# OpenGVLab/MM-Interleaved

Measured on NVIDIA H100. Metric: interleaved_steps_per_sec, higher is better.
Workload: dtype bf16

## Files before the change

### include/mmfs_b200.h

```cpp
#ifndef MMFS_B200_H_
#define MMFS_B200_H_

#include <stdint.h>

#ifdef __cplusplus
extern "C" {
#endif

#define MMFS_B200_ABI_VERSION 3

#define MMFS_OK            0
#define MMFS_EINVAL       (-1)
#define MMFS_EUNSUPPORTED (-2)
#define MMFS_ECUDA        (-3)

#define MMFS_F32  0
#define MMFS_F16  1
#define MMFS_BF16 2
#define MMFS_F64  3

#define MMFS_MSDA_STRICT 1u

#define MMFS_SAMPLER_EXACT_WEIGHTS 4u
#define MMFS_SAMPLER_GENERIC       8u
// ... 124 lines not shown
                       const float *params, const int64_t *seed, const float *uniforms, int B, int V, int max_new,
                       int mode, void *stream);

int mmfs_beam_select(const float *logits, long ld, const int64_t *step, const double *params, float *beam_scores,
                     int64_t *history, int64_t *next_ids, int64_t *parent, uint8_t *done, double *hyp_scores,
                     int64_t *hyp_ids, int64_t *hyp_meta, const int64_t *eos_ids, int n_eos, long pad_id, int min_length,
                     uint64_t *scratch, int B, int num_beams, int V, int max_new, void *stream);

int mmfs_beam_sample(const float *logits, long ld, const int64_t *step, const double *params, const int64_t *seed,
                     const float *uniforms, float *beam_scores, int64_t *history, int64_t *next_ids, int64_t *parent,
                     uint8_t *done, double *hyp_scores, int64_t *hyp_ids, int64_t *hyp_meta, int32_t *error,
                     const int64_t *eos_ids, int n_eos, long pad_id, int min_length, int top_k, uint64_t *scratch, int B,
                     int num_beams, int V, int max_new, void *stream);

int mmfs_kv_beam_reorder(void *cache, int n_caches, long cache_stride, int rows, long row_stride, long pos_stride,
                         long row_bytes, int num_beams, const int64_t *parent, const int64_t *cur, const int64_t *step,
                         const uint8_t *done, int max_positions, void *stream);

int mmfs_image_reentry(const float *images, float *out, int N, int C, int H, int W, int R, void *stream);

int mmfs_linear_fp8(const void *x, const uint8_t *w8, const float *scale, const void *bias, const void *residual,
                    void *out, int M, int N, int K, int dtype, void *stream);

#ifdef __cplusplus
}
#endif
#endif
```

### mm-interleaved_b200/_lib.py

```python
from __future__ import annotations

import ctypes
import os

_HERE = os.path.dirname(os.path.abspath(__file__))
LIB_PATH = os.environ.get("MMFS_B200_LIB", os.path.join(_HERE, "libmmfs_b200.so"))

OK, EINVAL, EUNSUPPORTED, ECUDA = 0, -1, -2, -3
F32, F16, BF16, F64 = 0, 1, 2, 3
MSDA_STRICT = 1
SAMPLER_EXACT_WEIGHTS = 4
SAMPLER_GENERIC = 8
SELECT_GREEDY, SELECT_SAMPLE = 0, 1

_lib = None

_I, _U, _P = ctypes.c_int, ctypes.c_uint, ctypes.c_void_p
_L, _F = ctypes.c_long, ctypes.c_float

SIGNATURES = {
    "mmfs_abi_version": (_I, []),
    "mmfs_last_error": (ctypes.c_char_p, []),
    "mmfs_msda_forward": (_I, [_P, _P, _P, _P, _P, _P, _I, _I, _I, _I, _I, _I, _I, _I, _U, _P]),
    "mmfs_msda_backward": (_I, [_P] * 9 + [_I] * 8 + [_P]),
# ... 13 lines not shown
    "mmfs_groupnorm_nhwc": (_I, [_P] * 5 + [_I] * 4 + [_F, _I, _I, _P]),
    "mmfs_groupnorm_nhwc_backward": (_I, [_P] * 6 + [_I] * 4 + [_F, _I, _I, _P]),
    "mmfs_conv2d_nhwc": (_I, [_P] * 6 + [_I] * 10 + [_P]),
    "mmfs_conv2d_up2x_nhwc": (_I, [_P] * 4 + [_I] * 6 + [_P]),
    "mmfs_conv2d_down2x_nhwc": (_I, [_P] * 4 + [_I] * 6 + [_P]),
    "mmfs_attn_decode_scratch_floats": (_L, [_I] * 4),
    "mmfs_attn_decode": (_I, [_P] * 6 + [_I] * 4 + [_L] * 6 + [_F, _I, _I, _I, _P]),
    "mmfs_attn_forward": (_I, [_P] * 5 + [_I] * 5 + [_L] * 8 + [_F, _I, _I, _I, _P, _P]),
    "mmfs_attn_forward_lse": (_I, [_P] * 6 + [_I] * 5 + [_L] * 8 + [_F, _I, _I, _I, _P, _P]),
    "mmfs_attn_backward": (_I, [_P] * 11 + [_I] * 4 + [_L] * 16 + [_F, _I, _P]),
    "mmfs_attn_backward_general": (_I, [_P] * 11 + [_I] * 5 + [_L] * 16 + [_F, _I, _I, _P]),
    "mmfs_rmsnorm_backward": (_I, [_P] * 6 + [_L, _I, _F, _I, _P]),
    "mmfs_layernorm_backward": (_I, [_P] * 7 + [_L, _I, _F, _I, _P]),
    "mmfs_swiglu_backward": (_I, [_P] * 3 + [_L, _I, _I, _P]),
    "mmfs_geglu_backward": (_I, [_P] * 3 + [_L, _I, _I, _P]),
    "mmfs_quick_gelu_backward": (_I, [_P] * 3 + [_L, _I, _P]),
    "mmfs_resize_bilinear_backward": (_I, [_P] * 2 + [_I] * 6 + [_L] * 3 + [_F, _F, _I, _P]),
    "mmfs_decode_select": (_I, [_P, _L] + [_P] * 5 + [_I, _L, _I] + [_P] * 3 + [_I] * 4 + [_P]),
    "mmfs_beam_select": (_I, [_P, _L] + [_P] * 11 + [_I, _L, _I, _P] + [_I] * 4 + [_P]),
    "mmfs_beam_sample": (_I, [_P, _L] + [_P] * 14 + [_I, _L, _I, _I, _P] + [_I] * 4 + [_P]),
    "mmfs_kv_beam_reorder": (_I, [_P, _I, _L, _I, _L, _L, _L, _I] + [_P] * 4 + [_I, _P]),
    "mmfs_image_reentry": (_I, [_P, _P] + [_I] * 5 + [_P]),
    "mmfs_linear_fp8": (_I, [_P] * 6 + [_I] * 4 + [_P]),
}
BEAM_MAX_BEAMS, BEAM_MAX_EOS = 8, 4
LINEAR_FP8_MAX_M = 64
RMSNORM_BWD_PARTS = 256


def lib() -> ctypes.CDLL:
    global _lib
    if _lib is None:
        if not os.path.exists(LIB_PATH):
            raise RuntimeError(
                f"libmmfs_b200.so not found at {LIB_PATH}: build it with "
                "`python mm-interleaved_b200/build.py` (there is no CPU / PyTorch fallback)")
        handle = ctypes.CDLL(LIB_PATH)
        for name, (res, args) in SIGNATURES.items():
            fn = getattr(handle, name)
            fn.restype = res
            fn.argtypes = args
        if handle.mmfs_abi_version() != 3:
            raise RuntimeError(f"libmmfs_b200.so ABI {handle.mmfs_abi_version()} != 3")
        _lib = handle
    return _lib

# ... 7 lines not shown
```

### mm-interleaved_b200/csrc/common.cuh

```cuda
#pragma once
#include <cuda_bf16.h>
#include <cuda_fp16.h>
#include <cuda_runtime.h>
#include <stdint.h>
#include <stdio.h>

#include <type_traits>

#include "../../include/mmfs_b200.h"

namespace mmfs {

void set_error(const char *fmt, ...);
int cuda_fail(cudaError_t e, const char *what);

#define MMFS_CHECK_ARG(cond, ...)            \
    do {                                     \
        if (!(cond)) {                       \
            ::mmfs::set_error(__VA_ARGS__);  \
            return MMFS_EINVAL;              \
        }                                    \
    } while (0)

#define MMFS_CUDA(call)                                             \
// ... 43 lines not shown
    MMFS_CUDA(cudaFuncSetAttribute(Kernel, cudaFuncAttributeMaxDynamicSharedMemorySize, (int)bytes));
    if (tracked) set[dev] = bytes;
    return MMFS_OK;
}

inline int capped_grid(long blocks, int per_sm) {
    const long cap = (long)num_sms() * per_sm;
    return (int)(blocks < cap ? blocks : cap);
}

template <typename T> struct OpMath { using type = float; };
template <> struct OpMath<double> { using type = double; };

__device__ __forceinline__ float to_op(float x) { return x; }
__device__ __forceinline__ double to_op(double x) { return x; }
__device__ __forceinline__ float to_op(__half x) { return __half2float(x); }
__device__ __forceinline__ float to_op(__nv_bfloat16 x) { return __bfloat162float(x); }

template <typename T> __device__ __forceinline__ T from_op(typename OpMath<T>::type x);
template <> __device__ __forceinline__ float from_op<float>(float x) { return x; }
template <> __device__ __forceinline__ double from_op<double>(double x) { return x; }
template <> __device__ __forceinline__ __half from_op<__half>(float x) { return __float2half_rn(x); }
template <> __device__ __forceinline__ __nv_bfloat16 from_op<__nv_bfloat16>(float x) { return __float2bfloat16_rn(x); }

template <typename T> struct Vec16;
template <> struct Vec16<float> {
    static constexpr int N = 4;
    __device__ __forceinline__ static void unpack(const uint4 &v, float (&f)[4]) {
        f[0] = __uint_as_float(v.x); f[1] = __uint_as_float(v.y);
        f[2] = __uint_as_float(v.z); f[3] = __uint_as_float(v.w);
    }
    __device__ __forceinline__ static uint4 pack(const float (&f)[4]) {
        return make_uint4(__float_as_uint(f[0]), __float_as_uint(f[1]), __float_as_uint(f[2]), __float_as_uint(f[3]));
    }
};
template <> struct Vec16<__nv_bfloat16> {
    static constexpr int N = 8;
    __device__ __forceinline__ static void unpack(const uint4 &v, float (&f)[8]) {
        f[0] = __uint_as_float(v.x << 16); f[1] = __uint_as_float(v.x & 0xffff0000u);
        f[2] = __uint_as_float(v.y << 16); f[3] = __uint_as_float(v.y & 0xffff0000u);
        f[4] = __uint_as_float(v.z << 16); f[5] = __uint_as_float(v.z & 0xffff0000u);
        f[6] = __uint_as_float(v.w << 16); f[7] = __uint_as_float(v.w & 0xffff0000u);
    }
    __device__ __forceinline__ static uint4 pack(const float (&f)[8]) {
        uint4 r;
        __nv_bfloat162 a = __floats2bfloat162_rn(f[0], f[1]); r.x = *reinterpret_cast<uint32_t *>(&a);
// ... 78 lines not shown
```

### mm-interleaved_b200/csrc/conv_igemm_sm100.cu

```cuda
#include "tc_common.cuh"

namespace mmfs {

constexpr int kConvStages = 4;
constexpr int kConvThreads = 288;
constexpr int kConvConsumers = 256;

struct ConvParams {
    void *out;
    const void *bias, *add_bc, *residual;
    int B, Ho, Wo, Cin, Cout, KH, KW, stride, pad;
    int TW, TH, TB;
    int tiles_w, tiles_h;
};

template <typename T> __device__ __forceinline__ uint32_t cpack2(float a, float b);
template <> __device__ __forceinline__ uint32_t cpack2<__nv_bfloat16>(float a, float b) {
    __nv_bfloat162 t = __floats2bfloat162_rn(a, b);
    return *reinterpret_cast<uint32_t *>(&t);
}
template <> __device__ __forceinline__ uint32_t cpack2<__half>(float a, float b) {
    __half2 t = __floats2half2_rn(a, b);
    return *reinterpret_cast<uint32_t *>(&t);
}
template <typename T> __device__ __forceinline__ float2 cunpack2(const T *p);
template <> __device__ __forceinline__ float2 cunpack2<__nv_bfloat16>(const __nv_bfloat16 *p) {
    return __bfloat1622float2(*reinterpret_cast<const __nv_bfloat162 *>(p));
}
template <> __device__ __forceinline__ float2 cunpack2<__half>(const __half *p) {
    return __half22float2(*reinterpret_cast<const __half2 *>(p));
}

template <typename T, int BN, bool UP>
__global__ void __launch_bounds__(kConvThreads, 1)
conv_igemm_kernel(const __grid_constant__ CUtensorMap map_x, const __grid_constant__ CUtensorMap map_w, const ConvParams p) {
    static_assert(BN == 160 || BN == 128, "Cout tile");
    constexpr uint32_t A_BYTES = 128 * 128, B_BYTES = BN * 128, STAGE_BYTES = A_BYTES + B_BYTES;
    extern __shared__ __align__(1024) uint8_t smem_raw[];
    if ((s_addr(smem_raw) & 1023u) != 0u) { asm volatile("trap;"); }
    uint64_t *bars = reinterpret_cast<uint64_t *>(smem_raw + kConvStages * STAGE_BYTES);
    uint64_t *full = bars, *empty = bars + kConvStages;

    const int warp = threadIdx.x >> 5, lane = threadIdx.x & 31;
    int t = blockIdx.x;
    const int wt = t % p.tiles_w; t /= p.tiles_w;
    const int ht = t % p.tiles_h; t /= p.tiles_h;
    const int b0 = t * p.TB, h0 = ht * p.TH, w0 = wt * p.TW;
// ... 181 lines not shown
```

### mm-interleaved_b200/csrc/llama_ops_sm100.cu

```cuda
#include "common.cuh"

namespace mmfs {

template <typename T> __device__ __forceinline__ float rnd(float x) { return to_op(from_op<T>(x)); }
template <> __device__ __forceinline__ float rnd<float>(float x) { return x; }

__device__ __forceinline__ float block_sum(float v, float *s_red) {
#pragma unroll
    for (int o = 16; o > 0; o >>= 1) v += __shfl_xor_sync(0xffffffffu, v, o);
    const int lane = threadIdx.x & 31, warp = threadIdx.x >> 5, nw = (blockDim.x + 31) >> 5;
    if (lane == 0) s_red[warp] = v;
    __syncthreads();
    float t = (lane < nw) ? s_red[lane] : 0.f;
#pragma unroll
    for (int o = 16; o > 0; o >>= 1) t += __shfl_xor_sync(0xffffffffu, t, o);
    __syncthreads();
    return t;
}

template <typename T>
__global__ void __launch_bounds__(256) rmsnorm_kernel(const T *__restrict__ x, const T *__restrict__ w,
                                                       T *__restrict__ y, int cols, float eps) {
    constexpr int VEC = 16 / (int)sizeof(T);
    __shared__ float s_red[32];
    const size_t row = blockIdx.x;
    const T *xr = x + row * cols;
    T *yr = y + row * cols;
    const int nvec = cols / VEC;
// ... 222 lines not shown
            const T *src = (is_k ? kt + (size_t)(hh - H) * hd : qt + (size_t)hh * hd) + c * VEC;
            T *dst = (is_k ? kc + (size_t)(hh - H) * hd : qt + (size_t)hh * hd) + c * VEC;
            float cs[VEC], sn[VEC], x1[VEC], x2[VEC], o1[VEC], o2[VEC];
#pragma unroll
            for (int i = 0; i < VEC; i += 4) {
                const float4 a = *reinterpret_cast<const float4 *>(cp + c * VEC + i);
                const float4 bb = *reinterpret_cast<const float4 *>(sp + c * VEC + i);
                cs[i] = rnd<T>(a.x); cs[i + 1] = rnd<T>(a.y); cs[i + 2] = rnd<T>(a.z); cs[i + 3] = rnd<T>(a.w);
                sn[i] = rnd<T>(bb.x); sn[i + 1] = rnd<T>(bb.y); sn[i + 2] = rnd<T>(bb.z); sn[i + 3] = rnd<T>(bb.w);
            }
            Vec16<T>::unpack(*reinterpret_cast<const uint4 *>(src), x1);
            Vec16<T>::unpack(*reinterpret_cast<const uint4 *>(src + half), x2);
#pragma unroll
            for (int i = 0; i < VEC; ++i) {
                o1[i] = rnd<T>(x1[i] * cs[i]) + rnd<T>(-x2[i] * sn[i]);
                o2[i] = rnd<T>(x2[i] * cs[i]) + rnd<T>(x1[i] * sn[i]);
            }
            *reinterpret_cast<uint4 *>(dst) = Vec16<T>::pack(o1);
            *reinterpret_cast<uint4 *>(dst + half) = Vec16<T>::pack(o2);
        }
    }
}

template <typename T> __device__ __forceinline__ float silu_op(float g) { return __fdividef(g, 1.f + __expf(-g)); }
template <> __device__ __forceinline__ float silu_op<float>(float g) { return g / (1.f + expf(-g)); }

template <typename T, int ACT> __device__ __forceinline__ float glu_act(float g) {
    if (ACT == 0) return silu_op<T>(g);
    return 0.5f * g * (1.f + erff(g * 0.70710678118654752f));
}

template <typename T, int ACT = 0, bool GATE_SECOND = false>
__global__ void __launch_bounds__(256) swiglu_kernel(const T *__restrict__ gu, T *__restrict__ out, long rows, int I) {
    constexpr int VEC = 16 / (int)sizeof(T);
    const int per = (I / VEC + gridDim.y - 1) / gridDim.y;
    const int v0 = blockIdx.y * per, nvec = min(I / VEC, v0 + per);
    for (long r = blockIdx.x; r < rows; r += gridDim.x) {
        const T *g_row = gu + r * 2 * I + (GATE_SECOND ? I : 0), *u_row = gu + r * 2 * I + (GATE_SECOND ? 0 : I);
        T *o_row = out + r * I;
        int i = v0 + threadIdx.x;
        for (; i + (int)blockDim.x < nvec; i += 2 * blockDim.x) {
            const int j = i + blockDim.x;
            const uint4 g0 = ldg_nc_v4(g_row + i * VEC), u0 = ldg_nc_v4(u_row + i * VEC);
            const uint4 g1 = ldg_nc_v4(g_row + j * VEC), u1 = ldg_nc_v4(u_row + j * VEC);
            float g[VEC], u[VEC], o[VEC];
            Vec16<T>::unpack(g0, g); Vec16<T>::unpack(u0, u);
#pragma unroll
            for (int k = 0; k < VEC; ++k) o[k] = rnd<T>(glu_act<T, ACT>(g[k])) * u[k];
            stg_v4(o_row + i * VEC, Vec16<T>::pack(o));
            Vec16<T>::unpack(g1, g); Vec16<T>::unpack(u1, u);
#pragma unroll
            for (int k = 0; k < VEC; ++k) o[k] = rnd<T>(glu_act<T, ACT>(g[k])) * u[k];
            stg_v4(o_row + j * VEC, Vec16<T>::pack(o));
        }
        if (i < nvec) {
            float g[VEC], u[VEC], o[VEC];
            Vec16<T>::unpack(ldg_nc_v4(g_row + i * VEC), g); Vec16<T>::unpack(ldg_nc_v4(u_row + i * VEC), u);
#pragma unroll
            for (int k = 0; k < VEC; ++k) o[k] = rnd<T>(glu_act<T, ACT>(g[k])) * u[k];
            stg_v4(o_row + i * VEC, Vec16<T>::pack(o));
        }
    }
}

template <typename T>
static int launch_rmsnorm(const void *x, const void *w, void *y, long rows, int cols, float eps, cudaStream_t st) {
    if (cols % (16 / (int)sizeof(T)) == 0 && cols / (16 / (int)sizeof(T)) <= kRmsThreads * kRmsChunks)
        rmsnorm_reg_kernel<T><<<(unsigned)rows, kRmsThreads, 0, st>>>((const T *)x, (const T *)w, (T *)y, cols, eps);
    else
        rmsnorm_kernel<T><<<(unsigned)rows, 256, 0, st>>>((const T *)x, (const T *)w, (T *)y, cols, eps);
    MMFS_CUDA(cudaGetLastError());
    return MMFS_OK;
}

template <typename T>
static int launch_layernorm(const void *x, const void *w, const void *b, void *y, long rows, int cols, float eps, cudaStream_t st) {
    constexpr int VEC = 16 / (int)sizeof(T);
    const bool vec_ok = (cols % VEC == 0) && (cols / VEC <= 32 * kLnChunks) &&
                        (((uintptr_t)x | (uintptr_t)y | (uintptr_t)w | (uintptr_t)b) % 16 == 0);
    if (vec_ok) {
        const int nvec = cols / VEC;
        const unsigned grid = (unsigned)((rows + 7) / 8);
// ... 453 lines not shown
```

### mm-interleaved_b200/csrc/tc_common.cuh

```cuda
#pragma once
#include <cuda.h>

#include "common.cuh"

namespace mmfs {

__device__ __forceinline__ void tma_load_4d(void *dst, const CUtensorMap *map, uint64_t *bar, int c0, int c1, int c2, int c3) {
    asm volatile(
        "cp.async.bulk.tensor.4d.shared::cluster.global.mbarrier::complete_tx::bytes [%0], [%1, {%3, %4, %5, %6}], [%2];" ::
        "r"(s_addr(dst)), "l"(map), "r"(s_addr(bar)), "r"(c0), "r"(c1), "r"(c2), "r"(c3) : "memory");
}
__device__ __forceinline__ void fence_async_smem() { asm volatile("fence.proxy.async.shared::cta;" ::: "memory"); }

__device__ __forceinline__ void wgmma_fence() { asm volatile("wgmma.fence.sync.aligned;" ::: "memory"); }
__device__ __forceinline__ void wgmma_commit() { asm volatile("wgmma.commit_group.sync.aligned;" ::: "memory"); }
template <int N> __device__ __forceinline__ void wgmma_wait() { asm volatile("wgmma.wait_group.sync.aligned %0;" ::"n"(N) : "memory"); }
template <int N> __device__ __forceinline__ void reg_fence(float (&d)[N]) {
#pragma unroll
    for (int i = 0; i < N; ++i) asm volatile("" : "+f"(d[i])::"memory");
}

__device__ __forceinline__ uint64_t smem_desc(uint32_t saddr, uint32_t lbo_bytes, uint32_t sbo_bytes) {
    return (uint64_t)((saddr >> 4) & 0x3fffu) | ((uint64_t)((lbo_bytes >> 4) & 0x3fffu) << 16) |
           ((uint64_t)((sbo_bytes >> 4) & 0x3fffu) << 32) | (1ull << 62);
}

template <typename T> struct Wgmma;
#define MMFS_WGMMA_OPS(TY) \
     \
// ... 1 lines not shown
        asm volatile( \
            "{\n\t.reg .pred p;\n\tsetp.ne.b32 p, %34, 0;\n\t" \
            "wgmma.mma_async.sync.aligned.m64n64k16.f32." TY "." TY " {%0,%1,%2,%3,%4,%5,%6,%7,%8,%9,%10,%11,%12,%13,%14,%15,%16,%17,%18,%19,%20,%21,%22,%23,%24,%25,%26,%27,%28,%29,%30,%31}, %32, %33, p, 1, 1, 0, 0;\n\t}" \
            : "+f"(d[0]), "+f"(d[1]), "+f"(d[2]), "+f"(d[3]), "+f"(d[4]), "+f"(d[5]), "+f"(d[6]), "+f"(d[7]), "+f"(d[8]), "+f"(d[9]), "+f"(d[10]), "+f"(d[11]), "+f"(d[12]), "+f"(d[13]), "+f"(d[14]), "+f"(d[15]), "+f"(d[16]), "+f"(d[17]), "+f"(d[18]), "+f"(d[19]), "+f"(d[20]), "+f"(d[21]), "+f"(d[22]), "+f"(d[23]), "+f"(d[24]), "+f"(d[25]), "+f"(d[26]), "+f"(d[27]), "+f"(d[28]), "+f"(d[29]), "+f"(d[30]), "+f"(d[31]) \
            : "l"(da), "l"(db), "r"(acc)); \
    } \
     \
    __device__ __forceinline__ static void ss_n128(float (&d)[64], uint64_t da, uint64_t db, int acc) { \
        asm volatile( \
            "{\n\t.reg .pred p;\n\tsetp.ne.b32 p, %66, 0;\n\t" \
            "wgmma.mma_async.sync.aligned.m64n128k16.f32." TY "." TY " {%0,%1,%2,%3,%4,%5,%6,%7,%8,%9,%10,%11,%12,%13,%14,%15,%16,%17,%18,%19,%20,%21,%22,%23,%24,%25,%26,%27,%28,%29,%30,%31,%32,%33,%34,%35,%36,%37,%38,%39,%40,%41,%42,%43,%44,%45,%46,%47,%48,%49,%50,%51,%52,%53,%54,%55,%56,%57,%58,%59,%60,%61,%62,%63}, %64, %65, p, 1, 1, 0, 0;\n\t}" \
            : "+f"(d[0]), "+f"(d[1]), "+f"(d[2]), "+f"(d[3]), "+f"(d[4]), "+f"(d[5]), "+f"(d[6]), "+f"(d[7]), "+f"(d[8]), "+f"(d[9]), "+f"(d[10]), "+f"(d[11]), "+f"(d[12]), "+f"(d[13]), "+f"(d[14]), "+f"(d[15]), "+f"(d[16]), "+f"(d[17]), "+f"(d[18]), "+f"(d[19]), "+f"(d[20]), "+f"(d[21]), "+f"(d[22]), "+f"(d[23]), "+f"(d[24]), "+f"(d[25]), "+f"(d[26]), "+f"(d[27]), "+f"(d[28]), "+f"(d[29]), "+f"(d[30]), "+f"(d[31]), "+f"(d[32]), "+f"(d[33]), "+f"(d[34]), "+f"(d[35]), "+f"(d[36]), "+f"(d[37]), "+f"(d[38]), "+f"(d[39]), "+f"(d[40]), "+f"(d[41]), "+f"(d[42]), "+f"(d[43]), "+f"(d[44]), "+f"(d[45]), "+f"(d[46]), "+f"(d[47]), "+f"(d[48]), "+f"(d[49]), "+f"(d[50]), "+f"(d[51]), "+f"(d[52]), "+f"(d[53]), "+f"(d[54]), "+f"(d[55]), "+f"(d[56]), "+f"(d[57]), "+f"(d[58]), "+f"(d[59]), "+f"(d[60]), "+f"(d[61]), "+f"(d[62]), "+f"(d[63]) \
            : "l"(da), "l"(db), "r"(acc)); \
    } \
     \
    __device__ __forceinline__ static void ss_n160(float (&d)[80], uint64_t da, uint64_t db, int acc) { \
        asm volatile( \
            "{\n\t.reg .pred p;\n\tsetp.ne.b32 p, %82, 0;\n\t" \
            "wgmma.mma_async.sync.aligned.m64n160k16.f32." TY "." TY " {%0,%1,%2,%3,%4,%5,%6,%7,%8,%9,%10,%11,%12,%13,%14,%15,%16,%17,%18,%19,%20,%21,%22,%23,%24,%25,%26,%27,%28,%29,%30,%31,%32,%33,%34,%35,%36,%37,%38,%39,%40,%41,%42,%43,%44,%45,%46,%47,%48,%49,%50,%51,%52,%53,%54,%55,%56,%57,%58,%59,%60,%61,%62,%63,%64,%65,%66,%67,%68,%69,%70,%71,%72,%73,%74,%75,%76,%77,%78,%79}, %80, %81, p, 1, 1, 0, 0;\n\t}" \
            : "+f"(d[0]), "+f"(d[1]), "+f"(d[2]), "+f"(d[3]), "+f"(d[4]), "+f"(d[5]), "+f"(d[6]), "+f"(d[7]), "+f"(d[8]), "+f"(d[9]), "+f"(d[10]), "+f"(d[11]), "+f"(d[12]), "+f"(d[13]), "+f"(d[14]), "+f"(d[15]), "+f"(d[16]), "+f"(d[17]), "+f"(d[18]), "+f"(d[19]), "+f"(d[20]), "+f"(d[21]), "+f"(d[22]), "+f"(d[23]), "+f"(d[24]), "+f"(d[25]), "+f"(d[26]), "+f"(d[27]), "+f"(d[28]), "+f"(d[29]), "+f"(d[30]), "+f"(d[31]), "+f"(d[32]), "+f"(d[33]), "+f"(d[34]), "+f"(d[35]), "+f"(d[36]), "+f"(d[37]), "+f"(d[38]), "+f"(d[39]), "+f"(d[40]), "+f"(d[41]), "+f"(d[42]), "+f"(d[43]), "+f"(d[44]), "+f"(d[45]), "+f"(d[46]), "+f"(d[47]), "+f"(d[48]), "+f"(d[49]), "+f"(d[50]), "+f"(d[51]), "+f"(d[52]), "+f"(d[53]), "+f"(d[54]), "+f"(d[55]), "+f"(d[56]), "+f"(d[57]), "+f"(d[58]), "+f"(d[59]), "+f"(d[60]), "+f"(d[61]), "+f"(d[62]), "+f"(d[63]), "+f"(d[64]), "+f"(d[65]), "+f"(d[66]), "+f"(d[67]), "+f"(d[68]), "+f"(d[69]), "+f"(d[70]), "+f"(d[71]), "+f"(d[72]), "+f"(d[73]), "+f"(d[74]), "+f"(d[75]), "+f"(d[76]), "+f"(d[77]), "+f"(d[78]), "+f"(d[79]) \
            : "l"(da), "l"(db), "r"(acc)); \
    } \
     \
    __device__ __forceinline__ static void rs_n64(float (&d)[32], const uint32_t (&a)[4], uint64_t db, int acc) { \
        asm volatile( \
            "{\n\t.reg .pred p;\n\tsetp.ne.b32 p, %37, 0;\n\t" \
            "wgmma.mma_async.sync.aligned.m64n64k16.f32." TY "." TY " {%0,%1,%2,%3,%4,%5,%6,%7,%8,%9,%10,%11,%12,%13,%14,%15,%16,%17,%18,%19,%20,%21,%22,%23,%24,%25,%26,%27,%28,%29,%30,%31}, {%32,%33,%34,%35}, %36, p, 1, 1, 1;\n\t}" \
            : "+f"(d[0]), "+f"(d[1]), "+f"(d[2]), "+f"(d[3]), "+f"(d[4]), "+f"(d[5]), "+f"(d[6]), "+f"(d[7]), "+f"(d[8]), "+f"(d[9]), "+f"(d[10]), "+f"(d[11]), "+f"(d[12]), "+f"(d[13]), "+f"(d[14]), "+f"(d[15]), "+f"(d[16]), "+f"(d[17]), "+f"(d[18]), "+f"(d[19]), "+f"(d[20]), "+f"(d[21]), "+f"(d[22]), "+f"(d[23]), "+f"(d[24]), "+f"(d[25]), "+f"(d[26]), "+f"(d[27]), "+f"(d[28]), "+f"(d[29]), "+f"(d[30]), "+f"(d[31]) \
            : "r"(a[0]), "r"(a[1]), "r"(a[2]), "r"(a[3]), "l"(db), "r"(acc)); \
    } \
     \
    __device__ __forceinline__ static void rs_n128(float (&d)[64], const uint32_t (&a)[4], uint64_t db, int acc) { \
        asm volatile( \
            "{\n\t.reg .pred p;\n\tsetp.ne.b32 p, %69, 0;\n\t" \
            "wgmma.mma_async.sync.aligned.m64n128k16.f32." TY "." TY " {%0,%1,%2,%3,%4,%5,%6,%7,%8,%9,%10,%11,%12,%13,%14,%15,%16,%17,%18,%19,%20,%21,%22,%23,%24,%25,%26,%27,%28,%29,%30,%31,%32,%33,%34,%35,%36,%37,%38,%39,%40,%41,%42,%43,%44,%45,%46,%47,%48,%49,%50,%51,%52,%53,%54,%55,%56,%57,%58,%59,%60,%61,%62,%63}, {%64,%65,%66,%67}, %68, p, 1, 1, 1;\n\t}" \
            : "+f"(d[0]), "+f"(d[1]), "+f"(d[2]), "+f"(d[3]), "+f"(d[4]), "+f"(d[5]), "+f"(d[6]), "+f"(d[7]), "+f"(d[8]), "+f"(d[9]), "+f"(d[10]), "+f"(d[11]), "+f"(d[12]), "+f"(d[13]), "+f"(d[14]), "+f"(d[15]), "+f"(d[16]), "+f"(d[17]), "+f"(d[18]), "+f"(d[19]), "+f"(d[20]), "+f"(d[21]), "+f"(d[22]), "+f"(d[23]), "+f"(d[24]), "+f"(d[25]), "+f"(d[26]), "+f"(d[27]), "+f"(d[28]), "+f"(d[29]), "+f"(d[30]), "+f"(d[31]), "+f"(d[32]), "+f"(d[33]), "+f"(d[34]), "+f"(d[35]), "+f"(d[36]), "+f"(d[37]), "+f"(d[38]), "+f"(d[39]), "+f"(d[40]), "+f"(d[41]), "+f"(d[42]), "+f"(d[43]), "+f"(d[44]), "+f"(d[45]), "+f"(d[46]), "+f"(d[47]), "+f"(d[48]), "+f"(d[49]), "+f"(d[50]), "+f"(d[51]), "+f"(d[52]), "+f"(d[53]), "+f"(d[54]), "+f"(d[55]), "+f"(d[56]), "+f"(d[57]), "+f"(d[58]), "+f"(d[59]), "+f"(d[60]), "+f"(d[61]), "+f"(d[62]), "+f"(d[63]) \
            : "r"(a[0]), "r"(a[1]), "r"(a[2]), "r"(a[3]), "l"(db), "r"(acc)); \
    }
template <> struct Wgmma<__nv_bfloat16> { MMFS_WGMMA_OPS("bf16") };
template <> struct Wgmma<__half> { MMFS_WGMMA_OPS("f16") };
#undef MMFS_WGMMA_OPS


__device__ __forceinline__ void tma_load_2d(void *dst, const CUtensorMap *map, uint64_t *bar, int c0, int c1) {
    asm volatile(
        "cp.async.bulk.tensor.2d.shared::cluster.global.mbarrier::complete_tx::bytes [%0], [%1, {%3, %4}], [%2];" ::
        "r"(s_addr(dst)), "l"(map), "r"(s_addr(bar)), "r"(c0), "r"(c1) : "memory");
}

typedef CUresult (*EncodeTiledFn)(CUtensorMap *, CUtensorMapDataType, cuuint32_t, void *, const cuuint64_t *, const cuuint64_t *,
                                  const cuuint32_t *, const cuuint32_t *, CUtensorMapInterleave, CUtensorMapSwizzle,
                                  CUtensorMapL2promotion, CUtensorMapFloatOOBfill);

inline EncodeTiledFn tensor_map_encoder() {
    static EncodeTiledFn fn = nullptr;
    if (!fn) {
        void *ptr = nullptr;
        cudaDriverEntryPointQueryResult qres;
        if (cudaGetDriverEntryPoint("cuTensorMapEncodeTiled", &ptr, cudaEnableDefault, &qres) == cudaSuccess &&
            qres == cudaDriverEntryPointSuccess)
            fn = (EncodeTiledFn)ptr;
    }
    return fn;
}

}
```

### mm-interleaved_b200/llama_mmfs.py

```python
from __future__ import annotations

import math
from dataclasses import dataclass, field
from types import SimpleNamespace
from typing import List, Optional, Tuple

import torch
import torch.nn.functional as F
from torch import nn

import torch.utils.checkpoint

from . import autograd_ops, ops
from ._cache import SourceCache, WeightCache
from .mmfs import MMFS
from .msda import records


@dataclass
class LlamaMMFSConfig:
    vocab_size: int = 32002
    hidden_size: int = 5120
    intermediate_size: int = 13824
    num_hidden_layers: int = 40
# ... 43 lines not shown

    def __init__(self, *linears):
        self.linears = linears
        self._cache = WeightCache()

    def get(self):
        ws = [l.weight for l in self.linears]
        if records(*ws):
            return torch.cat(ws, 0)
        return self._cache.get(ws, lambda: torch.cat(ws, 0).contiguous())


def _addmm_residual(residual, x, weight, inplace):
    r2 = residual.view(-1, residual.shape[-1])
    x2 = x.reshape(-1, x.shape[-1])
    if inplace:
        r2.addmm_(x2, weight.t())
        return residual
    return torch.addmm(r2, x2, weight.t()).view_as(residual)


FP8_DECODE_MAX_ROWS = 5


def decode_linear(x, weight, fp8, key, bias=None, residual=None, inplace=False):
    if (fp8 is not None and x.dim() == 3 and x.shape[1] == 1 and x.shape[0] <= FP8_DECODE_MAX_ROWS
            and weight.shape[0] >= 2 * weight.shape[1] and not records(x, residual)):
        w8, scale = fp8.get(weight, lambda: ops.quantize_fp8_per_channel(weight), key)
        return ops.linear_fp8(x, w8, scale, bias, residual, out=residual if inplace else None)
    if residual is None:
        return F.linear(x, weight, bias)
    return _addmm_residual(residual, x, weight, inplace)


class LlamaMLP(nn.Module):
    def __init__(self, hidden_size: int, intermediate_size: int, hidden_act: str):
        super().__init__()
        if hidden_act != "silu":
            raise NotImplementedError("only the SiLU gate of Llama is implemented")
        self.gate_proj = nn.Linear(hidden_size, intermediate_size, bias=False)
        self.down_proj = nn.Linear(intermediate_size, hidden_size, bias=False)
        self.up_proj = nn.Linear(hidden_size, intermediate_size, bias=False)
        self._gate_up = _CatWeight(self.gate_proj, self.up_proj)
        self._fp8 = None

    def forward(self, x, residual=None, inplace=False):
        gu = decode_linear(x, self._gate_up.get(), self._fp8, "gate_up")
        act = autograd_ops.swiglu(gu)
        return decode_linear(act, self.down_proj.weight, self._fp8, "down", residual=residual, inplace=inplace)


class StaticKV:

    __slots__ = ("k", "v", "length", "slot")

    def __init__(self, batch, max_len, heads, head_dim, dtype, device):
        self.k = torch.empty((batch, max_len, heads, head_dim), dtype=dtype, device=device)
        self.v = torch.empty_like(self.k)
        self.length = 0
        self.slot = None

    @classmethod
    def over(cls, k, v) -> "StaticKV":
        c = cls.__new__(cls)
        c.k, c.v, c.length, c.slot = k, v, 0, None
        return c


class PreparedVision:

    __slots__ = ("raw_shape", "values")
# ... 318 lines not shown
```

### mm-interleaved_b200/ops.py

```python
from __future__ import annotations

import math
from typing import Optional

import torch

from . import _lib
from .msda import _DTYPE_CODE, _require, inference_only

launch_counter = [0]


def _stream():
    return torch.cuda.current_stream().cuda_stream


def rmsnorm(x: torch.Tensor, weight: torch.Tensor, eps: float) -> torch.Tensor:
    inference_only("rmsnorm", x, weight)
    _require(x.is_cuda and x.is_contiguous() and weight.is_contiguous(), "rmsnorm: contiguous CUDA tensors required")
    _require(weight.dtype == x.dtype and weight.numel() == x.shape[-1], "rmsnorm: weight dtype / size mismatch")
    y = torch.empty_like(x)
    rows = x.numel() // x.shape[-1]
    with torch.cuda.device(x.device):
        rc = _lib.lib().mmfs_rmsnorm(x.data_ptr(), weight.data_ptr(), y.data_ptr(), rows, x.shape[-1], float(eps),
# ... 718 lines not shown
    N = w8.shape[0]
    _require(scale.dtype == torch.float32 and scale.is_contiguous() and scale.numel() == N and scale.device == x.device,
             f"linear_fp8: scale must be a contiguous fp32 tensor of {N} elements on {x.device}")
    _check_affine("linear_fp8", x, N, bias)
    x2 = x.reshape(-1, K)
    if not x2.is_contiguous() or x2.data_ptr() % 16:
        x2 = x2.clone(memory_format=torch.contiguous_format)
    M = x2.shape[0]
    shape = tuple(x.shape[:-1]) + (N,)
    for t, name in ((residual, "residual"), (out, "out")):
        if t is not None:
            _require(tuple(t.shape) == shape and t.dtype == x.dtype and t.is_contiguous() and t.device == x.device,
                     f"linear_fp8: {name} must be a contiguous {x.dtype} tensor of shape {shape}")
    if out is None:
        out = torch.empty(shape, dtype=x.dtype, device=x.device)
    with torch.cuda.device(x.device):
        rc = _lib.lib().mmfs_linear_fp8(x2.data_ptr(), w8.data_ptr(), scale.data_ptr(),
                                        bias.data_ptr() if bias is not None else None,
                                        residual.data_ptr() if residual is not None else None, out.data_ptr(),
                                        M, N, K, _DTYPE_CODE[x.dtype], _stream())
    _lib.check(rc, "linear_fp8")
    launch_counter[0] += 1
    return out
```

Baseline: 2.662.

## Fuse gate/up projection GEMM with SwiGLU in a clustered wgmma TMA kernel

Adds a warp-specialized Hopper GEMM kernel that computes the gate and up projections together and applies SwiGLU in the epilogue. A 2-CTA cluster multicasts the gate and up weight tiles so each CTA accumulates a 128x256 tile with m64n256k16 wgmma. The result is written through swizzled shared memory with TMA stores. The Llama MLP uses it for inputs of at least 1024 rows when not recording autograd. This avoids writing and re-reading the 2I-wide intermediate and a separate activation launch, in exchange for relying on a hand-written GEMM instead of cuBLAS.

```diff
diff --git a/include/mmfs_b200.h b/include/mmfs_b200.h
--- a/include/mmfs_b200.h
+++ b/include/mmfs_b200.h
@@ -170,6 +170,8 @@
 int mmfs_linear_fp8(const void *x, const uint8_t *w8, const float *scale, const void *bias, const void *residual,
                     void *out, int M, int N, int K, int dtype, void *stream);
 
+int mmfs_linear_swiglu(const void *x, const void *w_gu, void *out, int M, int I, int K, int plain, int dtype, void *stream);
+
 #ifdef __cplusplus
 }
 #endif
diff --git a/mm-interleaved_b200/_lib.py b/mm-interleaved_b200/_lib.py
--- a/mm-interleaved_b200/_lib.py
+++ b/mm-interleaved_b200/_lib.py
@@ -59,6 +59,7 @@
     "mmfs_kv_beam_reorder": (_I, [_P, _I, _L, _I, _L, _L, _L, _I] + [_P] * 4 + [_I, _P]),
     "mmfs_image_reentry": (_I, [_P, _P] + [_I] * 5 + [_P]),
     "mmfs_linear_fp8": (_I, [_P] * 6 + [_I] * 4 + [_P]),
+    "mmfs_linear_swiglu": (_I, [_P] * 3 + [_I] * 5 + [_P]),
 }
 BEAM_MAX_BEAMS, BEAM_MAX_EOS = 8, 4
 LINEAR_FP8_MAX_M = 64
diff --git a/mm-interleaved_b200/csrc/common.cuh b/mm-interleaved_b200/csrc/common.cuh
--- a/mm-interleaved_b200/csrc/common.cuh
+++ b/mm-interleaved_b200/csrc/common.cuh
@@ -89,6 +89,14 @@
 template <> __device__ __forceinline__ double from_op<double>(double x) { return x; }
 template <> __device__ __forceinline__ __half from_op<__half>(float x) { return __float2half_rn(x); }
 template <> __device__ __forceinline__ __nv_bfloat16 from_op<__nv_bfloat16>(float x) { return __float2bfloat16_rn(x); }
+
+template <typename T> __device__ __forceinline__ float rnd(float x) { return to_op(from_op<T>(x)); }
+template <> __device__ __forceinline__ float rnd<float>(float x) { return x; }
+
+template <typename T> __device__ __forceinline__ float silu_op(float g) { return __fdividef(g, 1.f + __expf(-g)); }
+template <> __device__ __forceinline__ float silu_op<float>(float g) { return g / (1.f + expf(-g)); }
+
+template <typename T> __device__ __forceinline__ float swiglu_op(float g, float u) { return rnd<T>(silu_op<T>(g)) * u; }
 
 template <typename T> struct Vec16;
 template <> struct Vec16<float> {
diff --git a/mm-interleaved_b200/csrc/conv_igemm_sm100.cu b/mm-interleaved_b200/csrc/conv_igemm_sm100.cu
--- a/mm-interleaved_b200/csrc/conv_igemm_sm100.cu
+++ b/mm-interleaved_b200/csrc/conv_igemm_sm100.cu
@@ -14,15 +14,6 @@
     int tiles_w, tiles_h;
 };
 
-template <typename T> __device__ __forceinline__ uint32_t cpack2(float a, float b);
-template <> __device__ __forceinline__ uint32_t cpack2<__nv_bfloat16>(float a, float b) {
-    __nv_bfloat162 t = __floats2bfloat162_rn(a, b);
-    return *reinterpret_cast<uint32_t *>(&t);
-}
-template <> __device__ __forceinline__ uint32_t cpack2<__half>(float a, float b) {
-    __half2 t = __floats2half2_rn(a, b);
-    return *reinterpret_cast<uint32_t *>(&t);
-}
 template <typename T> __device__ __forceinline__ float2 cunpack2(const T *p);
 template <> __device__ __forceinline__ float2 cunpack2<__nv_bfloat16>(const __nv_bfloat16 *p) {
     return __bfloat1622float2(*reinterpret_cast<const __nv_bfloat162 *>(p));
diff --git a/mm-interleaved_b200/csrc/gemm_swiglu_sm100.cu b/mm-interleaved_b200/csrc/gemm_swiglu_sm100.cu
--- /dev/null
+++ b/mm-interleaved_b200/csrc/gemm_swiglu_sm100.cu
@@ -0,0 +1,235 @@
+#include "tc_common.cuh"
+
+namespace mmfs {
+
+constexpr int kGsStages = 4;
+constexpr int kGsThreads = 384;
+constexpr int kGsCluster = 2;
+constexpr int kGsGroupPairs = 8;
+constexpr uint32_t kGsA = 128 * 128;
+constexpr uint32_t kGsBHalf = 128 * 128;
+constexpr uint32_t kGsStage = kGsA + 2 * kGsBHalf;
+constexpr uint32_t kGsOut = 64 * 128 * 2;
+constexpr size_t kGsSmem = (size_t)kGsStages * kGsStage + 2 * kGsOut + 2 * kGsStages * 8;
+
+struct GsParams {
+    int M, I, K;
+    int m_pairs, n_blocks, tiles;
+};
+
+__device__ __forceinline__ void gs_tile(int t, const GsParams &p, uint32_t rank, int &mb, int &nb) {
+    const int per_group = kGsGroupPairs * p.n_blocks;
+    const int g = t / per_group, r = t - g * per_group;
+    const int first = g * kGsGroupPairs, rows = min(kGsGroupPairs, p.m_pairs - first);
+    nb = r / rows;
+    mb = (first + r - nb * rows) * kGsCluster + (int)rank;
+}
+
+__device__ __forceinline__ void named_bar_sync(int id, int threads) {
+    asm volatile("bar.sync %0, %1;" ::"r"(id), "r"(threads) : "memory");
+}
+
+template <typename T, bool PLAIN>
+__global__ void __launch_bounds__(kGsThreads, 1)
+gemm_swiglu_kernel(const __grid_constant__ CUtensorMap map_x, const __grid_constant__ CUtensorMap map_w,
+                   const __grid_constant__ CUtensorMap map_out, const GsParams p) {
+    extern __shared__ __align__(1024) uint8_t smem[];
+    if ((s_addr(smem) & 1023u) != 0u) { asm volatile("trap;"); }
+    uint8_t *const out_stage = smem + kGsStages * kGsStage;
+    uint64_t *const full = reinterpret_cast<uint64_t *>(out_stage + 2 * kGsOut), *const empty = full + kGsStages;
+    const int wg = threadIdx.x >> 7, tid = threadIdx.x & 127, lane = threadIdx.x & 31;
+    const uint32_t rank = cluster_rank();
+    const int cluster_id = blockIdx.x / kGsCluster, n_clusters = gridDim.x / kGsCluster;
+    const int n_k = (p.K + 63) / 64;
+
+    if (threadIdx.x == 0) {
+        for (int i = 0; i < kGsStages; ++i) { bar_init(full + i, 1); bar_init(empty + i, 8 * kGsCluster); }
+        asm volatile("fence.mbarrier_init.release.cluster;" ::: "memory");
+    }
+    cluster_sync();
+
+    if (wg == 0) {
+        asm volatile("setmaxnreg.dec.sync.aligned.u32 40;");
+        if (tid == 0) {
+            int it = 0;
+            for (int t = cluster_id; t < p.tiles; t += n_clusters) {
+                int mb, nb;
+                gs_tile(t, p, rank, mb, nb);
+                for (int kb = 0; kb < n_k; ++kb, ++it) {
+                    const int s = it % kGsStages;
+                    bar_wait(empty + s, ((it / kGsStages) & 1) ^ 1);
+                    uint8_t *st = smem + s * kGsStage;
+                    bar_expect_tx(full + s, kGsStage);
+                    tma_load_2d(st, &map_x, full + s, kb * 64, mb * 128);
+                    tma_load_2d_multicast(st + kGsA + rank * kGsBHalf, &map_w, full + s, kb * 64,
+                                          (int)rank * p.I + nb * 128, (uint16_t)((1u << kGsCluster) - 1));
+                }
+            }
+        }
+        __syncwarp();
+    } else {
+        asm volatile("setmaxnreg.inc.sync.aligned.u32 232;");
+        const int c = wg - 1;
+        const int warp = (threadIdx.x >> 5) & 3;
+        uint8_t *const so = out_stage + c * kGsOut;
+        const uint32_t so_addr = s_addr(so);
+        float acc[128];
+        int it = 0;
+        auto release = [&](int s) {
+            __syncwarp();
+            if (lane == 0) {
+#pragma unroll
+                for (uint32_t r = 0; r < kGsCluster; ++r) bar_arrive_cluster(empty + s, r);
+            }
+        };
+        for (int t = cluster_id; t < p.tiles; t += n_clusters) {
+            int mb, nb;
+            gs_tile(t, p, rank, mb, nb);
+            for (int kb = 0; kb < n_k; ++kb, ++it) {
+                const int s = it % kGsStages;
+                bar_wait(full + s, (it / kGsStages) & 1);
+                const uint32_t sa = s_addr(smem) + s * kGsStage;
+                reg_fence(acc);
+                wgmma_fence();
+#pragma unroll
+                for (int kk = 0; kk < 4; ++kk) {
+                    const uint64_t da = smem_desc(sa + c * 64 * 128 + kk * 32, 16, 1024);
+                    const uint64_t db = smem_desc(sa + kGsA + kk * 32, 16, 1024);
+                    Wgmma<T>::ss_n256(acc, da, db, (kb | kk) != 0);
+                }
+                wgmma_commit();
+                wgmma_wait<1>();
+                reg_fence(acc);
+                if (kb > 0) release((it - 1) % kGsStages);
+            }
+            wgmma_wait<0>();
+            reg_fence(acc);
+            release((it - 1) % kGsStages);
+
+            const int row = mb * 128 + c * 64;
+#pragma unroll
+            for (int h = 0; h < (PLAIN ? 2 : 1); ++h) {
+                if (tid == 0) bulk_wait_read();
+                named_bar_sync(1 + c, 128);
+#pragma unroll
+                for (int j = 0; j < 16; ++j) {
+#pragma unroll
+                    for (int i = 0; i < 2; ++i) {
+                        const int a = 4 * (j + 16 * h) + 2 * i;
+                        uint32_t v;
+                        if constexpr (PLAIN) {
+                            v = cpack2<T>(acc[a], acc[a + 1]);
+                        } else {
+                            const float2 g = unpack2<T>(cpack2<T>(acc[a], acc[a + 1]));
+                            const float2 u = unpack2<T>(cpack2<T>(acc[a + 64], acc[a + 65]));
+                            v = cpack2<T>(swiglu_op<T>(g.x, u.x), swiglu_op<T>(g.y, u.y));
+                        }
+                        const int r = warp * 16 + (lane >> 2) + 8 * i;
+                        const uint32_t off = (j >> 3) * (64 * 128) + r * 128 + ((((uint32_t)j & 7u) ^ ((uint32_t)r & 7u)) << 4) +
+                                             (lane & 3) * 4;
+                        asm volatile("st.shared.u32 [%0], %1;" ::"r"(so_addr + off), "r"(v) : "memory");
+                    }
+                }
+                fence_async_smem();
+                named_bar_sync(1 + c, 128);
+                if (tid == 0) {
+                    if (row < p.M) {
+                        const int col = (PLAIN && h == 1 ? p.I : 0) + nb * 128;
+                        tma_store_2d(&map_out, so, col, row);
+                        tma_store_2d(&map_out, so + 64 * 128, col + 64, row);
+                    }
+                    bulk_commit();
+                }
+            }
+        }
+        if (tid == 0) bulk_wait();
+    }
+    cluster_sync();
+}
+
+}
+
+using namespace mmfs;
+
+namespace {
+
+template <auto kern>
+int gs_max_clusters(cudaLaunchConfig_t cfg, int *n) {
+    static int cached[kMaxDevices] = {};
+    const int dev = current_device();
+    if (dev >= 0 && dev < kMaxDevices && cached[dev] > 0) { *n = cached[dev]; return MMFS_OK; }
+    MMFS_CUDA(cudaOccupancyMaxActiveClusters(n, kern, &cfg));
+    if (*n <= 0) { set_error("linear_swiglu: no cluster of %d CTAs fits on the device", kGsCluster); return MMFS_EUNSUPPORTED; }
+    if (dev >= 0 && dev < kMaxDevices) cached[dev] = *n;
+    return MMFS_OK;
+}
+
+template <auto kern>
+int gs_launch(const CUtensorMap &mx, const CUtensorMap &mw, const CUtensorMap &mo, const GsParams &p, cudaStream_t st) {
+    int rc = ensure_dynamic_smem<kern>(kGsSmem);
+    if (rc != MMFS_OK) return rc;
+    cudaLaunchAttribute attr[1];
+    attr[0].id = cudaLaunchAttributeClusterDimension;
+    attr[0].val.clusterDim.x = kGsCluster;
+    attr[0].val.clusterDim.y = 1;
+    attr[0].val.clusterDim.z = 1;
+    cudaLaunchConfig_t cfg = {};
+    cfg.blockDim = dim3(kGsThreads);
+    cfg.dynamicSmemBytes = kGsSmem;
+    cfg.stream = st;
+    cfg.attrs = attr;
+    cfg.numAttrs = 1;
+    cfg.gridDim = dim3(kGsCluster);
+    int clusters = 0;
+    rc = gs_max_clusters<kern>(cfg, &clusters);
+    if (rc != MMFS_OK) return rc;
+    cfg.gridDim = dim3((unsigned)(kGsCluster * (clusters < p.tiles ? clusters : p.tiles)));
+    MMFS_CUDA(cudaLaunchKernelEx(&cfg, kern, mx, mw, mo, p));
+    return MMFS_OK;
+}
+
+int encode_2d(CUtensorMap *map, CUtensorMapDataType dt, const void *ptr, int cols, int rows, int box_cols, int box_rows,
+              CUtensorMapL2promotion l2, const char *what) {
+    EncodeTiledFn enc = tensor_map_encoder();
+    if (!enc) { set_error("linear_swiglu: cuTensorMapEncodeTiled unavailable"); return MMFS_ECUDA; }
+    const cuuint64_t dims[2] = {(cuuint64_t)cols, (cuuint64_t)rows};
+    const cuuint64_t strides[1] = {(cuuint64_t)cols * 2};
+    const cuuint32_t box[2] = {(cuuint32_t)box_cols, (cuuint32_t)box_rows};
+    const cuuint32_t estr[2] = {1, 1};
+    const CUresult r = enc(map, dt, 2, const_cast<void *>(ptr), dims, strides, box, estr, CU_TENSOR_MAP_INTERLEAVE_NONE,
+                           CU_TENSOR_MAP_SWIZZLE_128B, l2, CU_TENSOR_MAP_FLOAT_OOB_FILL_NONE);
+    if (r != CUDA_SUCCESS) { set_error("linear_swiglu: tensor map (%s) failed (%d)", what, (int)r); return MMFS_ECUDA; }
+    return MMFS_OK;
+}
+
+}
+
+extern "C" int mmfs_linear_swiglu(const void *x, const void *w_gu, void *out, int M, int I, int K, int plain, int dtype,
+                                  void *stream) {
+    MMFS_CHECK_ARG(M >= 0 && I > 0 && K > 0, "linear_swiglu: bad shape (M=%d I=%d K=%d)", M, I, K);
+    if (M == 0) return MMFS_OK;
+    MMFS_CHECK_ARG(x && w_gu && out, "linear_swiglu: null pointer argument");
+    if (!(dtype == MMFS_BF16 || dtype == MMFS_F16) || I % 128 != 0 || K % 8 != 0 ||
+        ((uintptr_t)x | (uintptr_t)w_gu | (uintptr_t)out) % 16 != 0) {
+        set_error("linear_swiglu: needs bf16 / f16, I %% 128 == 0, K %% 8 == 0 and 16-byte aligned pointers "
+                  "(I=%d K=%d dtype=%d)", I, K, dtype);
+        return MMFS_EUNSUPPORTED;
+    }
+    const CUtensorMapDataType dt = dtype == MMFS_BF16 ? CU_TENSOR_MAP_DATA_TYPE_BFLOAT16 : CU_TENSOR_MAP_DATA_TYPE_FLOAT16;
+    CUtensorMap mx, mw, mo;
+    int rc = encode_2d(&mx, dt, x, K, M, 64, 128, CU_TENSOR_MAP_L2_PROMOTION_L2_128B, "x");
+    if (rc == MMFS_OK) rc = encode_2d(&mw, dt, w_gu, K, 2 * I, 64, 128, CU_TENSOR_MAP_L2_PROMOTION_L2_256B, "w_gu");
+    if (rc == MMFS_OK) rc = encode_2d(&mo, dt, out, plain ? 2 * I : I, M, 64, 64, CU_TENSOR_MAP_L2_PROMOTION_NONE, "out");
+    if (rc != MMFS_OK) return rc;
+    GsParams p;
+    p.M = M; p.I = I; p.K = K;
+    p.m_pairs = (M + 128 * kGsCluster - 1) / (128 * kGsCluster);
+    p.n_blocks = I / 128;
+    p.tiles = p.m_pairs * p.n_blocks;
+    cudaStream_t st = (cudaStream_t)stream;
+    return dispatch_dtype<kF16Types>(dtype, "linear_swiglu", [&](auto tag) {
+        using T = typename decltype(tag)::type;
+        return plain ? gs_launch<gemm_swiglu_kernel<T, true>>(mx, mw, mo, p, st)
+                     : gs_launch<gemm_swiglu_kernel<T, false>>(mx, mw, mo, p, st);
+    });
+}
diff --git a/mm-interleaved_b200/csrc/llama_ops_sm100.cu b/mm-interleaved_b200/csrc/llama_ops_sm100.cu
--- a/mm-interleaved_b200/csrc/llama_ops_sm100.cu
+++ b/mm-interleaved_b200/csrc/llama_ops_sm100.cu
@@ -1,9 +1,6 @@
 #include "common.cuh"
 
 namespace mmfs {
-
-template <typename T> __device__ __forceinline__ float rnd(float x) { return to_op(from_op<T>(x)); }
-template <> __device__ __forceinline__ float rnd<float>(float x) { return x; }
 
 __device__ __forceinline__ float block_sum(float v, float *s_red) {
 #pragma unroll
@@ -272,12 +269,13 @@
     }
 }
 
-template <typename T> __device__ __forceinline__ float silu_op(float g) { return __fdividef(g, 1.f + __expf(-g)); }
-template <> __device__ __forceinline__ float silu_op<float>(float g) { return g / (1.f + expf(-g)); }
-
 template <typename T, int ACT> __device__ __forceinline__ float glu_act(float g) {
     if (ACT == 0) return silu_op<T>(g);
     return 0.5f * g * (1.f + erff(g * 0.70710678118654752f));
+}
+template <typename T, int ACT> __device__ __forceinline__ float glu_op(float g, float u) {
+    if (ACT == 0) return swiglu_op<T>(g, u);
+    return rnd<T>(glu_act<T, ACT>(g)) * u;
 }
 
 template <typename T, int ACT = 0, bool GATE_SECOND = false>
@@ -296,18 +294,18 @@
             float g[VEC], u[VEC], o[VEC];
             Vec16<T>::unpack(g0, g); Vec16<T>::unpack(u0, u);
 #pragma unroll
-            for (int k = 0; k < VEC; ++k) o[k] = rnd<T>(glu_act<T, ACT>(g[k])) * u[k];
+            for (int k = 0; k < VEC; ++k) o[k] = glu_op<T, ACT>(g[k], u[k]);
             stg_v4(o_row + i * VEC, Vec16<T>::pack(o));
             Vec16<T>::unpack(g1, g); Vec16<T>::unpack(u1, u);
 #pragma unroll
-            for (int k = 0; k < VEC; ++k) o[k] = rnd<T>(glu_act<T, ACT>(g[k])) * u[k];
+            for (int k = 0; k < VEC; ++k) o[k] = glu_op<T, ACT>(g[k], u[k]);
             stg_v4(o_row + j * VEC, Vec16<T>::pack(o));
         }
         if (i < nvec) {
             float g[VEC], u[VEC], o[VEC];
             Vec16<T>::unpack(ldg_nc_v4(g_row + i * VEC), g); Vec16<T>::unpack(ldg_nc_v4(u_row + i * VEC), u);
 #pragma unroll
-            for (int k = 0; k < VEC; ++k) o[k] = rnd<T>(glu_act<T, ACT>(g[k])) * u[k];
+            for (int k = 0; k < VEC; ++k) o[k] = glu_op<T, ACT>(g[k], u[k]);
             stg_v4(o_row + i * VEC, Vec16<T>::pack(o));
         }
     }
diff --git a/mm-interleaved_b200/csrc/tc_common.cuh b/mm-interleaved_b200/csrc/tc_common.cuh
--- a/mm-interleaved_b200/csrc/tc_common.cuh
+++ b/mm-interleaved_b200/csrc/tc_common.cuh
@@ -5,6 +5,22 @@
 
 namespace mmfs {
 
+template <typename T> __device__ __forceinline__ uint32_t cpack2(float a, float b);
+template <> __device__ __forceinline__ uint32_t cpack2<__nv_bfloat16>(float a, float b) {
+    __nv_bfloat162 t = __floats2bfloat162_rn(a, b);
+    return *reinterpret_cast<uint32_t *>(&t);
+}
+template <> __device__ __forceinline__ uint32_t cpack2<__half>(float a, float b) {
+    __half2 t = __floats2half2_rn(a, b);
+    return *reinterpret_cast<uint32_t *>(&t);
+}
+template <typename T> __device__ __forceinline__ float2 unpack2(uint32_t v);
+template <> __device__ __forceinline__ float2 unpack2<__nv_bfloat16>(uint32_t v) {
+    return make_float2(__uint_as_float(v << 16), __uint_as_float(v & 0xffff0000u));
+}
+template <> __device__ __forceinline__ float2 unpack2<__half>(uint32_t v) {
+    return __half22float2(*reinterpret_cast<const __half2 *>(&v));
+}
 __device__ __forceinline__ void tma_load_4d(void *dst, const CUtensorMap *map, uint64_t *bar, int c0, int c1, int c2, int c3) {
     asm volatile(
         "cp.async.bulk.tensor.4d.shared::cluster.global.mbarrier::complete_tx::bytes [%0], [%1, {%3, %4, %5, %6}], [%2];" ::
@@ -52,6 +68,14 @@
             : "l"(da), "l"(db), "r"(acc)); \
     } \
      \
+    __device__ __forceinline__ static void ss_n256(float (&d)[128], uint64_t da, uint64_t db, int acc) { \
+        asm volatile( \
+            "{\n\t.reg .pred p;\n\tsetp.ne.b32 p, %130, 0;\n\t" \
+            "wgmma.mma_async.sync.aligned.m64n256k16.f32." TY "." TY " {%0,%1,%2,%3,%4,%5,%6,%7,%8,%9,%10,%11,%12,%13,%14,%15,%16,%17,%18,%19,%20,%21,%22,%23,%24,%25,%26,%27,%28,%29,%30,%31,%32,%33,%34,%35,%36,%37,%38,%39,%40,%41,%42,%43,%44,%45,%46,%47,%48,%49,%50,%51,%52,%53,%54,%55,%56,%57,%58,%59,%60,%61,%62,%63,%64,%65,%66,%67,%68,%69,%70,%71,%72,%73,%74,%75,%76,%77,%78,%79,%80,%81,%82,%83,%84,%85,%86,%87,%88,%89,%90,%91,%92,%93,%94,%95,%96,%97,%98,%99,%100,%101,%102,%103,%104,%105,%106,%107,%108,%109,%110,%111,%112,%113,%114,%115,%116,%117,%118,%119,%120,%121,%122,%123,%124,%125,%126,%127}, %128, %129, p, 1, 1, 0, 0;\n\t}" \
+            : "+f"(d[0]), "+f"(d[1]), "+f"(d[2]), "+f"(d[3]), "+f"(d[4]), "+f"(d[5]), "+f"(d[6]), "+f"(d[7]), "+f"(d[8]), "+f"(d[9]), "+f"(d[10]), "+f"(d[11]), "+f"(d[12]), "+f"(d[13]), "+f"(d[14]), "+f"(d[15]), "+f"(d[16]), "+f"(d[17]), "+f"(d[18]), "+f"(d[19]), "+f"(d[20]), "+f"(d[21]), "+f"(d[22]), "+f"(d[23]), "+f"(d[24]), "+f"(d[25]), "+f"(d[26]), "+f"(d[27]), "+f"(d[28]), "+f"(d[29]), "+f"(d[30]), "+f"(d[31]), "+f"(d[32]), "+f"(d[33]), "+f"(d[34]), "+f"(d[35]), "+f"(d[36]), "+f"(d[37]), "+f"(d[38]), "+f"(d[39]), "+f"(d[40]), "+f"(d[41]), "+f"(d[42]), "+f"(d[43]), "+f"(d[44]), "+f"(d[45]), "+f"(d[46]), "+f"(d[47]), "+f"(d[48]), "+f"(d[49]), "+f"(d[50]), "+f"(d[51]), "+f"(d[52]), "+f"(d[53]), "+f"(d[54]), "+f"(d[55]), "+f"(d[56]), "+f"(d[57]), "+f"(d[58]), "+f"(d[59]), "+f"(d[60]), "+f"(d[61]), "+f"(d[62]), "+f"(d[63]), "+f"(d[64]), "+f"(d[65]), "+f"(d[66]), "+f"(d[67]), "+f"(d[68]), "+f"(d[69]), "+f"(d[70]), "+f"(d[71]), "+f"(d[72]), "+f"(d[73]), "+f"(d[74]), "+f"(d[75]), "+f"(d[76]), "+f"(d[77]), "+f"(d[78]), "+f"(d[79]), "+f"(d[80]), "+f"(d[81]), "+f"(d[82]), "+f"(d[83]), "+f"(d[84]), "+f"(d[85]), "+f"(d[86]), "+f"(d[87]), "+f"(d[88]), "+f"(d[89]), "+f"(d[90]), "+f"(d[91]), "+f"(d[92]), "+f"(d[93]), "+f"(d[94]), "+f"(d[95]), "+f"(d[96]), "+f"(d[97]), "+f"(d[98]), "+f"(d[99]), "+f"(d[100]), "+f"(d[101]), "+f"(d[102]), "+f"(d[103]), "+f"(d[104]), "+f"(d[105]), "+f"(d[106]), "+f"(d[107]), "+f"(d[108]), "+f"(d[109]), "+f"(d[110]), "+f"(d[111]), "+f"(d[112]), "+f"(d[113]), "+f"(d[114]), "+f"(d[115]), "+f"(d[116]), "+f"(d[117]), "+f"(d[118]), "+f"(d[119]), "+f"(d[120]), "+f"(d[121]), "+f"(d[122]), "+f"(d[123]), "+f"(d[124]), "+f"(d[125]), "+f"(d[126]), "+f"(d[127]) \
+            : "l"(da), "l"(db), "r"(acc)); \
+    } \
+     \
     __device__ __forceinline__ static void rs_n64(float (&d)[32], const uint32_t (&a)[4], uint64_t db, int acc) { \
         asm volatile( \
             "{\n\t.reg .pred p;\n\tsetp.ne.b32 p, %37, 0;\n\t" \
@@ -78,6 +102,34 @@
         "r"(s_addr(dst)), "l"(map), "r"(s_addr(bar)), "r"(c0), "r"(c1) : "memory");
 }
 
+__device__ __forceinline__ void tma_load_2d_multicast(void *dst, const CUtensorMap *map, uint64_t *bar, int c0, int c1,
+                                                      uint16_t mask) {
+    asm volatile(
+        "cp.async.bulk.tensor.2d.shared::cluster.global.mbarrier::complete_tx::bytes.multicast::cluster [%0], [%1, {%3, %4}], [%2], %5;" ::
+        "r"(s_addr(dst)), "l"(map), "r"(s_addr(bar)), "r"(c0), "r"(c1), "h"(mask) : "memory");
+}
+__device__ __forceinline__ void tma_store_2d(const CUtensorMap *map, const void *src, int c0, int c1) {
+    asm volatile("cp.async.bulk.tensor.2d.global.shared::cta.bulk_group [%0, {%2, %3}], [%1];" ::
+                 "l"(map), "r"(s_addr(src)), "r"(c0), "r"(c1) : "memory");
+}
+__device__ __forceinline__ void bulk_commit() { asm volatile("cp.async.bulk.commit_group;" ::: "memory"); }
+__device__ __forceinline__ void bulk_wait_read() { asm volatile("cp.async.bulk.wait_group.read 0;" ::: "memory"); }
+__device__ __forceinline__ void bulk_wait() { asm volatile("cp.async.bulk.wait_group 0;" ::: "memory"); }
+
+__device__ __forceinline__ uint32_t cluster_rank() {
+    uint32_t r;
+    asm volatile("mov.u32 %0, %%cluster_ctarank;" : "=r"(r));
+    return r;
+}
+__device__ __forceinline__ void cluster_sync() {
+    asm volatile("barrier.cluster.arrive.release.aligned;\n\tbarrier.cluster.wait.acquire.aligned;" ::: "memory");
+}
+__device__ __forceinline__ void bar_arrive_cluster(uint64_t *bar, uint32_t rank) {
+    asm volatile(
+        "{\n\t.reg .b32 a;\n\tmapa.shared::cluster.u32 a, %0, %1;\n\t"
+        "mbarrier.arrive.shared::cluster.b64 _, [a];\n\t}" ::"r"(s_addr(bar)), "r"(rank) : "memory");
+}
+
 typedef CUresult (*EncodeTiledFn)(CUtensorMap *, CUtensorMapDataType, cuuint32_t, void *, const cuuint64_t *, const cuuint64_t *,
                                   const cuuint32_t *, const cuuint32_t *, CUtensorMapInterleave, CUtensorMapSwizzle,
                                   CUtensorMapL2promotion, CUtensorMapFloatOOBfill);
diff --git a/mm-interleaved_b200/llama_mmfs.py b/mm-interleaved_b200/llama_mmfs.py
--- a/mm-interleaved_b200/llama_mmfs.py
+++ b/mm-interleaved_b200/llama_mmfs.py
@@ -89,6 +89,8 @@
 
 FP8_DECODE_MAX_ROWS = 5
 
+LINEAR_SWIGLU_MIN_ROWS = 1024
+
 
 def decode_linear(x, weight, fp8, key, bias=None, residual=None, inplace=False):
     if (fp8 is not None and x.dim() == 3 and x.shape[1] == 1 and x.shape[0] <= FP8_DECODE_MAX_ROWS
@@ -112,8 +114,13 @@
         self._fp8 = None
 
     def forward(self, x, residual=None, inplace=False):
-        gu = decode_linear(x, self._gate_up.get(), self._fp8, "gate_up")
-        act = autograd_ops.swiglu(gu)
+        w_gu = self._gate_up.get()
+        if (x.numel() >= LINEAR_SWIGLU_MIN_ROWS * x.shape[-1] and not records(x, w_gu)
+                and ops.linear_swiglu_supported(x, w_gu)):
+            act = ops.linear_swiglu(x, w_gu)
+        else:
+            gu = decode_linear(x, w_gu, self._fp8, "gate_up")
+            act = autograd_ops.swiglu(gu)
         return decode_linear(act, self.down_proj.weight, self._fp8, "down", residual=residual, inplace=inplace)
 
 
diff --git a/mm-interleaved_b200/ops.py b/mm-interleaved_b200/ops.py
--- a/mm-interleaved_b200/ops.py
+++ b/mm-interleaved_b200/ops.py
@@ -764,3 +764,37 @@
     _lib.check(rc, "linear_fp8")
     launch_counter[0] += 1
     return out
+
+
+def linear_swiglu_supported(x: torch.Tensor, w_gu: torch.Tensor) -> bool:
+    K = x.shape[-1]
+    return (x.is_cuda and x.dtype in (torch.bfloat16, torch.float16) and w_gu.dtype == x.dtype
+            and w_gu.device == x.device and w_gu.dim() == 2 and w_gu.shape[1] == K and K % 8 == 0
+            and w_gu.shape[0] % 256 == 0 and w_gu.shape[0] > 0)
+
+
+def _linear_gate_up(x: torch.Tensor, w_gu: torch.Tensor, plain: bool) -> torch.Tensor:
+    inference_only("linear_swiglu", x, w_gu)
+    _require(linear_swiglu_supported(x, w_gu),
+             "linear_swiglu: needs CUDA bf16 / fp16 x (..., K) and w_gu (2I, K) of the same dtype and device, "
+             "I % 128 == 0, K % 8 == 0")
+    K, I = x.shape[-1], w_gu.shape[0] // 2
+    x2 = x.reshape(-1, K)
+    if not x2.is_contiguous() or x2.data_ptr() % 16:
+        x2 = x2.clone(memory_format=torch.contiguous_format)
+    w = w_gu if w_gu.is_contiguous() and w_gu.data_ptr() % 16 == 0 else w_gu.contiguous()
+    out = torch.empty(tuple(x.shape[:-1]) + ((2 * I) if plain else I,), dtype=x.dtype, device=x.device)
+    with torch.cuda.device(x.device):
+        rc = _lib.lib().mmfs_linear_swiglu(x2.data_ptr(), w.data_ptr(), out.data_ptr(), x2.shape[0], I, K, int(plain),
+                                           _DTYPE_CODE[x.dtype], _stream())
+    _lib.check(rc, "linear_swiglu")
+    launch_counter[0] += 1
+    return out
+
+
+def linear_swiglu(x: torch.Tensor, w_gu: torch.Tensor) -> torch.Tensor:
+    return _linear_gate_up(x, w_gu, False)
+
+
+def linear_gate_up_plain(x: torch.Tensor, w_gu: torch.Tensor) -> torch.Tensor:
+    return _linear_gate_up(x, w_gu, True)
```

Measured after the change: 2.698 (median of 6 runs). 1.4% higher.
